# madsim-rs/madsim

Hardware: AMD Instinct MI355X
Metric: sim_seconds_per_sec (higher is better)
Workload: dtype u64

## Files before the change

madsim_amd/csrc/kernel/k_channel.h:

```cpp
#ifndef MADSIM_K_CHANNEL_H
#define MADSIM_K_CHANNEL_H

namespace madsim_k {

template <class K>
__device__ __forceinline__ int net_try_send(const Ctx& c, Lane& L, uint32_t src_node, uint32_t addr, uint32_t idx, uint64_t* latency, int* dst_sock, uint32_t* from_lb, uint32_t* dst_hdr,
                                            uint32_t known_idx = ~0u, uint32_t known_hdr = 0) {
    const KParams& P = c.P;
    int res = 0;
    uint32_t hdr = 0;
    if (K::G && PLAIN_ADDR) {
        if (idx == known_idx) {
#ifdef MADSIM_EMU
            if (known_hdr != (uint32_t)SW(c, idx, 0)) OVF_SET(L, OVF_BUG);
#endif
            hdr = known_hdr;
        } else hdr = SW(c, idx, 0);
    }
    int dn = (int)(addr & 0xff);
    if (!PLAIN_ADDR) dn = resolve_dest_node<K>(c, src_node, addr);
    if (dn >= 0) {
        const uint32_t dst_node = (uint32_t)dn;
        bool clogged = false;
        const bool mir = K::LIFE && MADSIM_CLOG_MIRROR;
        if (P.has_clog && (!mir || (L.loss_always & 0x100u))) clogged = ((CLOGW(1) >> src_node) & 1) | ((CLOGW(0) >> dst_node) & 1);
        if (P.has_clog_link && (!mir || (L.loss_always & 0x200u))) clogged |= (CLOGW(2 + src_node) >> dst_node) & 1;
        if (!clogged && !gen_bool_pint<K>(c, L, L.loss_pint, K::LIFE ? (L.loss_always & 1u) : L.loss_always)) {
            L.msg_count++;
            *latency = sample_latency<K>(c, L);
            int ds;
            if (PLAIN_ADDR) { if (!K::G) hdr = SW(c, idx, 0); ds = (hdr & 1) ? (int)idx : -1; }
            else {
                ds = find_exact<K>(c, dst_node, addr);
                if (ds < 0) ds = find_exact<K>(c, dst_node, (addr & 0xffff0000u) | (MADSIM_ADDR_UNSPECIFIED << 8));
                if (ds >= 0) hdr = SW(c, (uint32_t)ds, 0);
            }
            if (ds >= 0) {
                *from_lb = 0;
                res = 1;
                if (!PLAIN_ADDR) {
                    *from_lb = ((addr >> 8) & 0xff) == MADSIM_ADDR_LOOPBACK;
// ... 115 lines not shown
```

madsim_amd/csrc/kernel/k_lifecycle.h:

```cpp
#ifndef MADSIM_K_LIFECYCLE_H
#define MADSIM_K_LIFECYCLE_H

namespace madsim_k {

struct SpawnInit { bool parent_known; uint32_t parent_f, parent_u1y; bool move_req; uint32_t w, from, req;
                   bool words_known; uint32_t slot, w_old, w_gen, seq, w_killed; };
template <class K>
__device__ __forceinline__ uint32_t spawn_task(const Ctx& c, Lane& L, uint32_t prog, bool record, bool via_handle = false, int parent = -1,
                                               const SpawnInit init = SpawnInit{false, 0, 0, false, 0, 0, 0, false, 0, 0, 0, 0, 0}) {
    uint32_t slot = 0;
    if (K::G) {
        slot = c.P.max_tasks;
        if (init.words_known) slot = init.slot;
        else for (uint32_t wi = 0; wi < (c.P.max_tasks + 31) / 32; wi++) {
            uint32_t free_bits = ~AMASK(wi);
            if (free_bits) { slot = wi * 32 + (uint32_t)__builtin_ctz(free_bits); break; }
        }
#ifdef MADSIM_EMU
        if (init.words_known && ((AMASK(slot >> 5) >> (slot & 31)) & 1)) OVF_SET(L, OVF_BUG);
#endif
    } else {
        while (slot < c.P.max_tasks && (TWORD(c, slot, 0, 0) & TF_ALIVE)) slot++;
    }
    if (slot >= c.P.max_tasks) { OVF_SET(L, c.P.max_tasks >= MADSIM_MAX_LIVE_TASKS ? OVF_MODEL : OVF_CAP); return 0xffffffffu; }
    if (K::G) AMASK(slot >> 5) |= 1u << (slot & 31);
    uint32_t pw, node, gen, killed = 0, info_gen = 0, seq = 0;
    if constexpr (K::G) {
        pw = PROGW(c, prog);
        node = pw & 0xff;
        uint32_t w_old = init.w_old;
        uint32_t w_gen = init.w_gen, w_parent_f = init.parent_f, w_parent_y = init.parent_u1y, w_killed = init.w_killed;
        const bool in_parent = parent >= 0;
        seq = init.seq;
        if (!init.words_known) {
            w_old = TWORD(c, slot, 0, 0);
            if (K::FN) {
                w_gen = NODEW(4 + (node >> 2));
                seq = NODEW(3);
                if (!in_parent) w_killed = NODEW(via_handle ? 2u : 0u);
// ... 67 lines not shown
            uint32_t m = OMASK(wi);
            while (m) {
                uint32_t ix[4], ow[4], n = 0;
                for (uint32_t k = 0; k < 4; k++) { ix[k] = wi * 32 + (uint32_t)__builtin_ctz(m | 0x80000000u); if (m) { n++; m &= m - 1; } }
                for (uint32_t k = 0; k < 4; k++) ow[k] = SW(c, k < n ? ix[k] : ix[0], 1);
                for (uint32_t k = 0; k < 4; k++) {
                    if (k >= n || ow[k] != key) continue;
                    const uint32_t i = ix[k];
                    OMASK(i >> 5) &= ~(1u << (i & 31));
                    endpoint_drop<K>(c, L, i, (f & TF_KILLED) != 0);
                    if (SW(c, i, 1) != ~0u) SW(c, i, 1) = 0x0000ff00u;
                }
            }
        }
    } else if (f & TF_OWNER) {
        for (uint32_t i = 0; i < c.P.n_socks; i++) {
            const uint32_t hdr = SW(c, i, 0);
            if (!sock_owned_by<K>(c, i, hdr, slot, gen)) continue;
            endpoint_drop<K>(c, L, i, (f & TF_KILLED) != 0);
            if (K::LIFE && SW(c, i, 1) != ~0u) SW(c, i, 1) = 0x0000ff00u;
        }
    }
}

template <class K>
__device__ __forceinline__ void task_drop_guard(const Ctx& c, Lane& L, uint32_t slot, uint32_t prog) {
    if (K::FN && K::FA && ((PROGW(c, prog) >> 8) & MADSIM_PROG_DROP_SPAWN)) spawn_task<K>(c, L, prog + 1, false, false, (int)slot);
}

struct FinishKnown { bool have; uint32_t f, link, cx; bool have_h; uint32_t h; };
template <class K>
// ... 166 lines not shown
```

madsim_amd/csrc/kernel/k_main.h:

```cpp
#ifndef MADSIM_K_MAIN_H
#define MADSIM_K_MAIN_H

namespace madsim_k {

template <class K>
__device__ __forceinline__ void seed_init(const Ctx& c, Lane& L, uint64_t seed) {
    const KParams& P = c.P;
    if (K::G) {
        for (uint32_t w = 0; w < P.gs_plane_words; w++) gs_store32(c.gs, gs_addr_word(c, P.gs_planes + w * 4), 0);
        for (uint32_t w = 0; w < (P.max_tasks + 31) / 32; w++) AMASK(w) = 0;
        OMASK(0) = 0; OMASK(1) = 0;
        if (K::NH) for (uint32_t w = 0; w < P.pool_n / 32; w++) PMASK(w) = 0;
    }
    else for (uint32_t w = 0; w < P.lane_words; w++) RW(w) = 0;
    if (K::DEDUP) { for (uint32_t b = 0; b < P.dedup_n; b++) gs_store32(c.gs, gs_addr_uword(c, P.dedup_off + b * 16u + 12u), 0); L.hazard = 0; L.dd_occ = 0; }
    for (uint32_t t = 0; t < P.max_tasks; t++) { TWORD(c, t, 0, 0) = 0; if (!K::LIFE) TWORD(c, t, 1, 1) = 0; }
    if (K::FA && P.ipvs_dyn)
        for (uint32_t k = 0; k < P.n_services; k++) {
            const uint32_t w0 = SMEM[c.nodet0 + P.svc_off + 2 * k], w1 = SMEM[c.nodet0 + P.svc_off + 2 * k + 1];
            IPVSW(2 * k) = (w0 >> 16) | (w1 << 16);
            IPVSW(2 * k + 1) = (w1 >> 16) | (((w0 >> 8) & 7u) << 16) | ((w0 & 0x8000u) ? 0u : 1u << 24);
        }
    uint64_t x = seed, z;
#define SPLITMIX(dst) x += 0x9e3779b97f4a7c15ull; z = x; z = (z ^ (z >> 30)) * 0xbf58476d1ce4e5b9ull; z = (z ^ (z >> 27)) * 0x94d049bb133111ebull; dst = z ^ (z >> 31)
    SPLITMIX(L.s0); SPLITMIX(L.s1); SPLITMIX(L.s2); SPLITMIX(L.s3);
#undef SPLITMIX
    L.peek = rng_out(L);
    L.rng_calls = 0; L.clock = 0; L.msg_count = 0; L.steps = 0;
    L.pq_n = 0; L.ready_len = 0; L.rq = 0; L.heap_len = 0; L.top_dl = ~0ull; L.top_meta = 0; L.verdict = MADSIM_RUNNING; L.ovf = 0; L.main_done = 0;
    L.loss_pint = P.loss_pint; L.loss_always = P.loss_always;
    L.clock_fold = 0;
    { uint64_t h = L.trace_hash, n = L.log_len; uint32_t bt = gen_range_small<Variant<false, false, K::LWS, 0, K::RQ>, 31536000u>(c, L); L.trace_hash = h; L.log_len = n;
      if (K::LIFE) NODEW(4 + ((P.n_nodes + 4) >> 2)) = bt; }
    L.trace_hash = FNV_OFFSET; L.obs_hash = FNV_OFFSET; L.log_len = 0;
    if (K::TRACE) L.obs_len = 0;
    for (uint32_t p = 1; p < P.n_progs; p++) {
        uint32_t fl = (PROGW(c, p) >> 8) & 0xff;
        if (fl & MADSIM_PROG_PRE) spawn_task<K>(c, L, p, !(fl & MADSIM_PROG_INIT));
    }
    spawn_task<K>(c, L, 0, true);
}

#ifndef MADSIM_G_WAVES_PER_EU
#define MADSIM_G_WAVES_PER_EU 3
#endif
#ifndef MADSIM_ALLG_WAVES_PER_EU
#define MADSIM_ALLG_WAVES_PER_EU 2
#endif
constexpr uint32_t MADSIM_PRIO_EVERY_MASK = 15u;
__device__ __forceinline__ uint32_t progress_priority(uint32_t pass, uint32_t est) {
    const uint32_t q = (pass < (1u << 30) ? pass : (1u << 30) - 1u) * 4u / est;
    return q >= 3 ? 0u : 3u - q;
}

template <class K> struct PopOne { static constexpr bool ON = MADSIM_POP_ONE && K::RQ; };

template <class K>
__global__ __launch_bounds__(256, K::CMP ? 4 : !K::G ? 1 : (K::FEAT & (MADSIM_FEAT_ALL & ~MADSIM_FEAT_ADDR)) == (MADSIM_FEAT_ALL & ~MADSIM_FEAT_ADDR) ? MADSIM_ALLG_WAVES_PER_EU : MADSIM_G_WAVES_PER_EU) void sim_kernel(const KParams P) {
    const uint32_t lane = threadIdx.x & 63, wv = threadIdx.x >> 6;
    uint32_t* sh = SMEM;
    const uint32_t cp0 = table_copy_first(), cps = table_copy_stride(P.waves_per_block);
    for (uint32_t i = cp0; i < P.n_insns * 4; i += cps) sh[P.sh_insns + i] = ((const uint32_t*)P.insns)[i];
    for (uint32_t i = cp0; i < P.n_progs; i += cps) sh[P.sh_progs + i] = P.progs[i];
    for (uint32_t i = cp0; i < P.n_socks; i += cps) sh[P.sh_socks + i] = P.socks[i];
    for (uint32_t i = cp0; i < P.n_nodetab; i += cps) sh[P.sh_nodes + i] = P.nodes[i];
    __syncthreads();

    Ctx c(P);
    c.insn0 = P.sh_insns / 4;
    c.prog0 = P.sh_progs;
    c.sockt0 = P.sh_socks;
    c.nodet0 = P.sh_nodes;
    const uint32_t wbase = wv * P.wave_words;
    if (K::NH) c.heap0 = (P.sh_heap + wbase) / 2 + lane;
    else if (K::LIFE) c.heap0 = (P.sh_heap + wbase) / 4 + lane;
    else if (K::CMP) { c.heap0 = (P.sh_heap + wbase) / 2 + lane; c.heapm0 = 0; }
    else { c.heap0 = (P.sh_heap + wbase) / 2 + lane; c.heapm0 = P.sh_heap + wbase + ((P.heap_lds * 2) << P.lw_shift) + lane; }
    c.lws = P.lw_shift;
    const uint32_t pl = P.sh_planes + wbase + lane;
    c.ready0 = pl + (P.off_ready << P.lw_shift);
    c.amask0 = pl + (P.off_amask << P.lw_shift);
    c.omask0 = pl + (P.off_omask << P.lw_shift);
    c.pmask0 = pl + (P.off_pmask << P.lw_shift);
    if (K::G) {
        c.task0 = 0;
        c.sock0 = P.gs_planes + P.off_socks * 4; c.hand0 = P.gs_planes + P.off_handles * 4; c.node0 = P.gs_planes + P.off_nodes * 4;
        c.clog0 = P.gs_planes + P.off_clog * 4; c.pause0 = P.gs_planes + P.off_pause * 4; c.greg0 = P.gs_planes + P.off_greg * 4;
        c.conn0 = P.gs_planes + P.off_conn * 4; c.hook0 = P.gs_planes + P.off_hooks * 4; c.ipvs0 = P.gs_planes + P.off_ipvs * 4;
    } else {
        c.task0 = (P.sh_tasks + wbase) / 4 + lane;
        c.task1 = (P.sh_tasks + wbase + ((P.max_tasks * 4) << P.lw_shift)) / 2 + lane;
        if (K::CMP) {
            c.task1 = (P.sh_tasks + wbase + (((P.max_tasks - 1) * 4) << P.lw_shift)) / 2 + lane - (1u << P.lw_shift);
// ... 17 lines not shown
    c.gs_lane = glane;
    c.gs = buf_make(P.gstate, (uint64_t)P.gs_stride * P.total_lanes);
    c.tlog = P.trace_log;

    Lane L;
#ifdef MADSIM_K_PROF
    for (int i = 0; i < 12; i++) L.prof_acc[i] = 0;
    L.prof_t = __builtin_readcyclecounter(); uint64_t prof_iters = 0;
#endif
    L.exact = 0; L.hazard = 0;
    uint64_t next = glane;
    bool have = false;
    uint32_t pass_est = (K::TRACE || !P.iter_est) ? 0u : wave_uniform(*P.iter_est);
    uint32_t pass = 0;
    for (;;) {
        if (!K::TRACE && P.iter_est) {
            const uint32_t pu = wave_uniform(pass);
            if ((pu & MADSIM_PRIO_EVERY_MASK) == 0) {
                if (!pass_est && (pu & 63u) == 0) pass_est = wave_uniform(__atomic_load_n(P.iter_est, __ATOMIC_RELAXED));
                if (pass_est) wave_set_priority(progress_priority(pu, pass_est));
            }
        }
        pass++;
        if (!have) {
            if (next >= P.count) break;
            if (K::TRACE) {
                c.tlog = P.trace_log + next * P.trace_cap;
                c.olog = (P.obs_log && P.obs_cap) ? P.obs_log + next * P.obs_cap : nullptr;
            }
            seed_init<K>(c, L, P.seed_list ? P.seed_list[next] : P.seed0 + next);
            have = true;
        }
#ifdef MADSIM_K_PROF
        prof_iters++;
#endif
        uint64_t now = L.clock;
        PROBE(0);
        REG(0);
        if (L.ready_len > 0) {
            const uint32_t slot0 = K::RQ ? (uint32_t)(L.rq & 0xff) : rq_get<K>(c, 0);
            const uint4 pu0 = TU(c, slot0, 0), pu1 = load_u1<K>(c, slot0);
            PollPrefetch pp = poll_prefetch<K>(c, slot0);
            if (ClockFold<K>::ON) L.clock_fold = clock_fold_byte(L.clock);
            const bool all_one = wave_all(L.ready_len == 1);
            uint32_t idx = gen_index<K>(c, L, L.ready_len, all_one);
// ... 84 lines not shown
            }
            L.verdict = v;
            if (v != MADSIM_RUNNING || more) break;
            now = L.top_dl + 50;
            idle_jump = true;
        }
        PROBE(4);
        if (K::DEDUP && L.hazard) { L.exact = 1; have = false; continue; }
        if (L.ovf) L.verdict = (L.ovf & OVF_CAP) ? MADSIM_OVERFLOW : (L.ovf & OVF_BUG) ? MADSIM_INTERNAL : MADSIM_UNSUPPORTED;
        if (L.verdict != MADSIM_RUNNING) {
            REG(25);
            madsim_result_t r;
            r.verdict = L.verdict; r.steps = L.steps; r.clock_ns = L.clock; r.msg_count = L.msg_count;
            r.rng_calls = L.rng_calls; r.trace_hash = (K::NOLOG || (K::LOGSW && P.no_log)) ? 0 : L.trace_hash; r.obs_hash = L.obs_hash;
            if (r.verdict >= MADSIM_UNSUPPORTED) { r.steps = 0; r.clock_ns = 0; r.msg_count = 0; r.rng_calls = 0; r.trace_hash = 0; r.obs_hash = 0; }
            P.out[next] = r;
            if (K::TRACE) { P.trace_len[next] = L.log_len; if (P.obs_len) P.obs_len[next] = L.obs_len; }
            have = false;
            if (K::DEDUP) L.exact = 0;
            if (P.work_ctr) next = P.total_lanes + atomicAdd(P.work_ctr, 1ull);
            else next += P.total_lanes / EXP_LANE_DIV;
        }
    }
    if (!K::TRACE && P.iter_est) {
        if (K::LIFE) {
            const uint32_t wmax = wave_max_u32(pass);
            if (wave_first_lane() && wmax > 16) atomic_max_u32(P.iter_est, wmax);
        } else if (lane == 0 && pass > 16) *P.iter_est = pass;
    }
#ifdef MADSIM_K_PROF
    PROBE2(0);
    if (lane == 0 && P.prof) { for (int i = 0; i < 12; i++) atomicAdd((unsigned long long*)&P.prof[i], (unsigned long long)L.prof_acc[i]); atomicAdd((unsigned long long*)&P.prof[12], (unsigned long long)prof_iters); atomicAdd((unsigned long long*)&P.prof[13], 1ull); }
#endif
}

}

#endif
```

madsim_amd/csrc/kernel/k_poll.h:

```cpp
#ifndef MADSIM_K_POLL_H
#define MADSIM_K_POLL_H

namespace madsim_k {

__device__ __forceinline__ uint64_t sleep_deadline(const Lane& L, uint64_t deadline) {
    uint64_t m = L.clock + NS_PER_MS;
    return deadline > m ? deadline : m;
}

template <class K>
__device__ __forceinline__ uint64_t rand_delay_deadline(const Ctx& c, Lane& L) {
    uint64_t delay = (uint64_t)gen_range_small<K, 5>(c, L) * 1000ull;
    if (c.P.buggify) {
        if (gen_bool_pint<K>(c, L, c.P.bug_pint, 0)) delay = (uint64_t)(1 + gen_range_small<K, 4>(c, L)) * NS_PER_S;
    }
    return sleep_deadline(L, L.clock + delay);
}

__device__ __forceinline__ uint64_t loss_pint_at(const KParams& P, uint32_t i) {
    i &= 3;
    return i == 0 ? P.loss_table_pint[0] : i == 1 ? P.loss_table_pint[1] : i == 2 ? P.loss_table_pint[2] : P.loss_table_pint[3];
}
__device__ __forceinline__ uint32_t loss_always_at(const KParams& P, uint32_t i) {
    i &= 3;
    return i == 0 ? P.loss_table_always[0] : i == 1 ? P.loss_table_always[1] : i == 2 ? P.loss_table_always[2] : P.loss_table_always[3];
}

__device__ __forceinline__ bool may_have_twin(uint32_t flags, uint32_t gen) { return (flags & TF_RXWRAP) || gen > 0xff; }
// ... 46 lines not shown
        u0.w = MADSIM_VAL_TIMEOUT;
        return true;
    }
    timer_schedule<K>(c, L, dl, (EV_WAKE << EV_SHIFT) | (gen << 8) | slot, 0, true, again);
    return false;
}

__device__ __forceinline__ bool is_light(uint32_t op) {
    return op == MS_OP_ASSERT_VAL || op == MS_OP_DJNZ || op == MS_OP_SET || op == MS_OP_JMP || op == MS_OP_TRACE || op == MS_OP_JEQ;
}

template <class K>
__device__ __forceinline__ bool poll_task(const Ctx& c, Lane& L, const uint32_t slot, uint4& u0, uint4 u1, PollPrefetch pp) {
    enum : uint32_t { ST_RUN = 0, ST_PENDING = 1, ST_FINISHED = 2, ST_PANIC = 3 };
    const KParams& P = c.P;
    const uint32_t REGS_FULL = P.mbox_regs >= MADSIM_MAX_MBOX_REGS ? (uint32_t)OVF_MODEL : (uint32_t)OVF_CAP;
    bool u1_dirty = false;
    uint32_t pc = u0.y & 0xffff, sub = (u0.y >> 16) & 0xff, from = u0.y >> 24;
    const uint32_t gen = (u0.x >> 8) & 0xffff;
    const uint32_t node = PROGW(c, u0.x >> 24) & 0xff;
    uint32_t st = ST_RUN;
    bool sig = false;
    if constexpr (K::FSIG) { sig = (sub & SUB_SIGNALLED) != 0; sub &= ~SUB_SIGNALLED; }

    bool first_poll = false;
    constexpr bool CU_FULL = Hoist<K>::CHAN;
    auto cu_get = [&]() -> uint4 { if (CU_FULL) return pp.cu; return (uint4)TU(c, slot, c.P.chan_unit); };
    auto cu0_get = [&]() -> uint32_t { if (K::G) return pp.cu.x; return (uint32_t)TWORD(c, slot, c.P.chan_unit, 0); };
    auto cu0_set = [&](uint32_t v) { if (K::G) pp.cu.x = v; TWORD(c, slot, c.P.chan_unit, 0) = v; };
    auto cu_set = [&](const uint4& v) { if (CU_FULL) pp.cu = v; else if (K::G) pp.cu.x = v.x; TU(c, slot, c.P.chan_unit) = v; };
#ifdef MADSIM_EMU
// ... 627 lines not shown
                    if (K::FR && P.uses_rpc && (b & MADSIM_SPAWN_MOVE_REQUEST) && child != 0xffffffffu) {
                        TWORD(c, child, 0, 3) = u0.w;
                        TWORD(c, child, 0, 1) = (TWORD(c, child, 0, 1) & 0x00ffffffu) | (from << 24);
                        TWORD(c, child, P.rpc_unit, 0) = TWORD(c, slot, P.rpc_unit, 0);
                    }
                }
                if (K::FC && P.uses_chan && (b & 2) && child != 0xffffffffu) {
                    uint32_t cx = cu0_get();
                    TWORD(c, child, c.P.chan_unit, 0) = cx & 0x1ff;
                    cu0_set(cx | 0xff);
                }
            }
                pc++;
                break;
            case MS_OP_BUILD:
                for (uint32_t p = 1; p < P.n_progs; p++) {
                    uint32_t pw = PROGW(c, p);
                    if ((pw & 0xff) == a && ((pw >> 8) & MADSIM_PROG_INIT) && !((pw >> 8) & MADSIM_PROG_PRE)) spawn_task<K>(c, L, p, false);
                }
                pc++;
                break;
            case MS_OP_JOIN: {
                uint32_t hs;
                if (sub == SUB_JOIN_WAIT) { st = ST_PENDING; break; }
                if (sub != 0) { hs = sub == SUB_JOIN_CANCELLED ? H_CANCELLED : H_COMPLETED; sub = 0; }
                else {
                    const uint32_t h = HW(a);
                    hs = h & 3;
                    if (hs == H_RUNNING) {
                        const uint32_t cs = (h >> 8) & 0xff;
                        const uint32_t link = TWORD(c, cs, 1, 0);
// ... 294 lines not shown
            REG(17);
            u1.z = (uint32_t)deadline; u1.w = (uint32_t)(deadline >> 32); u1_dirty = true;
            sub = (op == MS_OP_RECV) ? 3 : 1;
            timer_schedule<K>(c, L, deadline, (EV_WAKE << EV_SHIFT) | (gen << 8) | slot, 0, true);
            st = ST_PENDING;
        }
    }
    PROBE(9);
    if (st != ST_FINISHED) {
        u0.y = pc | (sub << 16) | (from << 24);
        if (u1_dirty) tu1_store<K>(c, slot, u1);
    }
    return st == ST_PANIC;
}
#undef RX_DROP
#undef SCOPE_DROP_CONN

}

#endif
```

madsim_amd/csrc/kernel/k_state.h:

```cpp
#ifndef MADSIM_K_STATE_H
#define MADSIM_K_STATE_H

namespace madsim_k {

#ifdef MADSIM_EXPERIMENT_BUILD
#include <type_traits>
#include "../../../tools/experiment/k_experiment.h"
#else
#if defined(EXP_NOLOG) || defined(EXP_ALWAYS_ACCEPT) || defined(EXP_PROF) || defined(EXP_PROF2) || defined(EXP_NO_LWS_VARIANTS) || defined(EXP_HALF_LANES)
#error "EXP_* switches make a non-bit-exact kernel: build experiment variants with tools/build_variant.sh, never the product Makefile"
#endif
#define EXP_ACCEPT(x) (x)
#define EXP_LANE_DIV 1u
#define MADSIM_K_LOG_ENABLED 1
#define PROBE(i) do { } while (0)
#define PROBE2(i) do { } while (0)
#define PROBE_FLUSH() do { } while (0)
#endif
#define FNV_OFFSET 14695981039346656037ull
#define FNV_PRIME 1099511628211ull
#define NS_PER_S 1000000000ull
#define NS_PER_MS 1000000ull

enum : uint32_t { TF_ALIVE = 1, TF_SCHED = 2, TF_RUN = 4, TF_KILLED = 8, TF_CANCEL = 16, TF_INBOX = 32,
// ... 14 lines not shown
    static constexpr int LWS = LWS_, FEAT = FEAT_ & MADSIM_FEAT_ALL;
    static constexpr bool LIFE = FEAT != 0;
    static constexpr bool CMP = (FEAT_ & MADSIM_FEAT_COMPACT) != 0;
    static constexpr bool NOLOG = (FEAT_ & MADSIM_FEAT_NOLOG) != 0;
    static constexpr bool NH = (FEAT_ & MADSIM_FEAT_NARROW) != 0;
    static constexpr bool LOGSW = !NOLOG && !TRACE_ && (LIFE || SPILL_ || LWS_ != 6);
    static constexpr bool DEDUP = G_ && !TRACE_ && (FEAT_ & MADSIM_FEAT_ALL) == MADSIM_FEAT_TIME;
    static constexpr bool FT = (FEAT_ & MADSIM_FEAT_TIME) != 0, FC = (FEAT_ & MADSIM_FEAT_CHAN) != 0,
                          FR = (FEAT_ & MADSIM_FEAT_RPC) != 0, FN = (FEAT_ & MADSIM_FEAT_NODE) != 0,
                          FA = (FEAT_ & MADSIM_FEAT_ADDR) != 0;
    static constexpr bool FS = (FEAT_ & MADSIM_FEAT_SCOPE) != 0;
    static constexpr bool FK = (FEAT_ & MADSIM_FEAT_TICK) != 0;
    static constexpr bool FSEL = (FEAT_ & MADSIM_FEAT_SELECT) != 0;
    static constexpr bool FSIG = (FEAT_ & MADSIM_FEAT_SIGNAL) != 0;
};

#ifndef REG
#define REG(id) do { } while (0)
#endif

enum : uint32_t { OVF_CAP = 1, OVF_MODEL = 2, OVF_BUG = 4 };
#ifdef MADSIM_EMU
void madsim_emu_ovf_note(const char* file, int line, uint32_t bits);
#define OVF_SET(L, bits) ((L).ovf = (L).ovf ? (L).ovf : (bits), madsim_emu_ovf_note(__FILE__, __LINE__, (bits)))
#else
#define OVF_SET(L, bits) ((L).ovf = (L).ovf ? (L).ovf : (bits))
#endif
struct Lane {
    uint64_t s0, s1, s2, s3;
    uint64_t peek;
// ... 37 lines not shown
    uint32_t sock0;
    uint32_t heap0;
    uint32_t heapm0;
    uint32_t task0;
    uint32_t task1;
    uint32_t insn0;
    uint32_t prog0, sockt0, nodet0;
    BufRef spill;
    uint32_t spill_off;
    BufRef gs;
    uint32_t gs_lane;
    uint32_t amask0, omask0;
    uint32_t pmask0;
    uint8_t* tlog;
    uint64_t* olog;
    __device__ Ctx(const KParams& p) : P(p) {}
};

template <class K> __device__ __forceinline__ uint32_t LWSH(const Ctx& c) { return K::LWS >= 0 ? (uint32_t)K::LWS : c.lws; }
#define RW(i) SMEM[c.ready0 + ((i) << LWSH<K>(c))]
template <class K> __device__ __forceinline__ uint32_t rq_get(const Ctx& c, uint32_t i) {
    if (!K::G) return RW(i);
    return (RW(i >> 2) >> ((i & 3u) * 8u)) & 0xffu;
}
template <class K> __device__ __forceinline__ void rq_set(const Ctx& c, uint32_t i, uint32_t slot) {
    if (!K::G) { RW(i) = slot; return; }
    const uint32_t sh = (i & 3u) * 8u, w = RW(i >> 2);
    RW(i >> 2) = (w & ~(0xffu << sh)) | (slot << sh);
}
#define AMASK(i) SMEM[c.amask0 + ((i) << LWSH<K>(c))]
#define OMASK(i) SMEM[c.omask0 + ((i) << LWSH<K>(c))]
#define PMASK(i) SMEM[c.pmask0 + ((i) << LWSH<K>(c))]

// ... 25 lines not shown
    __device__ __forceinline__ uint32_t operator+=(uint32_t v) const { return *this = (uint32_t)*this + v; }
};
template <bool G> struct URef;
template <> struct URef<false> {
    uint32_t at;
    __device__ __forceinline__ operator uint4() const { return LDS128(at); }
    __device__ __forceinline__ void operator=(const uint4& v) const { LDS128(at) = v; }
    __device__ __forceinline__ void operator=(const URef& o) const { *this = (uint4)o; }
};
template <> struct URef<true> {
    BufRef gs; uint32_t at;
    __device__ __forceinline__ operator uint4() const { return gs_load128(gs, at); }
    __device__ __forceinline__ void operator=(const uint4& v) const { gs_store128(gs, at, v); }
    __device__ __forceinline__ void operator=(const URef& o) const { *this = (uint4)o; }
};
struct HWRef {
    BufRef gs; uint32_t at; bool glob;
    __device__ __forceinline__ operator uint32_t() const { uint32_t v; if (glob) v = gs_load32(gs, at); else v = SMEM[at]; return v; }
    __device__ __forceinline__ uint32_t operator=(uint32_t v) const { if (glob) gs_store32(gs, at, v); else SMEM[at] = v; return v; }
    __device__ __forceinline__ uint32_t operator=(const HWRef& o) const { return *this = (uint32_t)o; }
    __device__ __forceinline__ uint32_t operator|=(uint32_t v) const { return *this = (uint32_t)*this | v; }
    __device__ __forceinline__ uint32_t operator&=(uint32_t v) const { return *this = (uint32_t)*this & v; }
    __device__ __forceinline__ uint32_t operator+=(uint32_t v) const { return *this = (uint32_t)*this + v; }
};
struct HURef {
    BufRef gs; uint32_t at; bool glob;
    __device__ __forceinline__ operator uint4() const { uint4 v; if (glob) v = gs_load128(gs, at); else v = LDS128(at); return v; }
    __device__ __forceinline__ void operator=(const uint4& v) const { if (glob) gs_store128(gs, at, v); else LDS128(at) = v; }
    __device__ __forceinline__ void operator=(const HURef& o) const { *this = (uint4)o; }
};
template <class K> struct TaskRef {
    typedef typename std::conditional<K::CMP, HURef, URef<K::G>>::type U;
    typedef typename std::conditional<K::CMP, HWRef, WRef<K::G>>::type W;
};
template <bool G> __device__ __forceinline__ WRef<G> make_wref(const Ctx& c, uint32_t lds_at, uint32_t gs_at);
template <> __device__ __forceinline__ WRef<false> make_wref<false>(const Ctx&, uint32_t lds_at, uint32_t) { return WRef<false>{lds_at}; }
__device__ __forceinline__ uint32_t gs_addr_unit(const Ctx& c, uint32_t at) { return __umul24(at, c.P.total_lanes) + c.gs_lane * 16u; }
__device__ __forceinline__ uint32_t gs_addr_uword(const Ctx& c, uint32_t at) { return __umul24(at & ~15u, c.P.total_lanes) + c.gs_lane * 16u + (at & 15u); }
__device__ __forceinline__ uint32_t gs_addr_word(const Ctx& c, uint32_t at) { return __umul24(at, c.P.total_lanes) + c.gs_lane * 4u; }
template <> __device__ __forceinline__ WRef<true> make_wref<true>(const Ctx& c, uint32_t, uint32_t gs_at) { return WRef<true>{c.gs, gs_addr_word(c, gs_at)}; }
__device__ __forceinline__ WRef<true> make_uword_ref(const Ctx& c, uint32_t gs_at) { return WRef<true>{c.gs, gs_addr_uword(c, gs_at)}; }
template <bool G> __device__ __forceinline__ URef<G> make_uref(const Ctx& c, uint32_t lds_at, uint32_t gs_at);
template <> __device__ __forceinline__ URef<false> make_uref<false>(const Ctx&, uint32_t lds_at, uint32_t) { return URef<false>{lds_at}; }
template <> __device__ __forceinline__ URef<true> make_uref<true>(const Ctx& c, uint32_t, uint32_t gs_at) { return URef<true>{c.gs, gs_addr_unit(c, gs_at)}; }
template <class K> __device__ __forceinline__ WRef<K::G> plane_ref(const Ctx& c, uint32_t base, uint32_t i) {
    return make_wref<K::G>(c, base + (i << LWSH<K>(c)), base + i * 4u);
}
#define NODEW(i) plane_ref<K>(c, c.node0, (i))
// ... 27 lines not shown
template <> __device__ __forceinline__ URef<false> tu_gs<false>(const Ctx&, uint32_t, uint32_t) { return URef<false>{0}; }
template <> __device__ __forceinline__ URef<true> tu_gs<true>(const Ctx& c, uint32_t slot, uint32_t u) { return URef<true>{c.gs, gs_addr_task(c, slot, u * 16u)}; }
template <bool G> __device__ __forceinline__ WRef<G> tword_gs2(const Ctx& c, uint32_t slot, uint32_t u, uint32_t k);
template <> __device__ __forceinline__ WRef<false> tword_gs2<false>(const Ctx&, uint32_t, uint32_t, uint32_t) { return WRef<false>{0}; }
template <> __device__ __forceinline__ WRef<true> tword_gs2<true>(const Ctx& c, uint32_t slot, uint32_t u, uint32_t k) { return WRef<true>{c.gs, gs_addr_task(c, slot, u * 16u + k * 4u)}; }
template <class K> __device__ __forceinline__ URef<K::G> tu_ref_plain(const Ctx& c, uint32_t slot, uint32_t u) {
    if (!K::LIFE) return make_uref<K::G>(c, c.task0 + (slot << LWSH<K>(c)), 0);
    if (K::G) return tu_gs<K::G>(c, slot, u);
    return make_uref<K::G>(c, c.task0 + ((slot * c.P.task_units + u) << LWSH<K>(c)), 0);
}
template <class K> __device__ __forceinline__ WRef<K::G> tword_ref_plain(const Ctx& c, uint32_t slot, uint32_t u, uint32_t k) {
    if (!K::LIFE) return make_wref<K::G>(c, u == 0 ? (c.task0 + (slot << LWSH<K>(c))) * 4u + k : (c.task1 + (slot << LWSH<K>(c))) * 2u + k, 0);
    if (K::G) return tword_gs2<K::G>(c, slot, u, k);
    return make_wref<K::G>(c, (c.task0 + ((slot * c.P.task_units + u) << LWSH<K>(c))) * 4u + k, 0);
}
template <class K> __device__ __forceinline__ typename TaskRef<K>::U tu_ref(const Ctx& c, uint32_t slot, uint32_t u) {
    if constexpr (K::CMP) return HURef{c.gs, slot == 0 ? c.gs_lane * 16u : c.task0 + (slot << LWSH<K>(c)), slot == 0};
    else return tu_ref_plain<K>(c, slot, u);
}
template <class K> __device__ __forceinline__ typename TaskRef<K>::W tword_ref(const Ctx& c, uint32_t slot, uint32_t u, uint32_t k) {
    if constexpr (K::CMP) {
        const uint32_t lds = u == 0 ? (c.task0 + (slot << LWSH<K>(c))) * 4u + k : (c.task1 + (slot << LWSH<K>(c))) * 2u + k;
        const uint32_t glb = u == 0 ? c.gs_lane * 16u + k * 4u : c.P.total_lanes * 16u + c.gs_lane * 8u + k * 4u;
        return HWRef{c.gs, slot == 0 ? glb : lds, slot == 0};
    } else return tword_ref_plain<K>(c, slot, u, k);
}
template <class K> __device__ __forceinline__ uint4 load_u1(const Ctx& c, uint32_t slot) {
    if (K::LIFE) return tu_ref<K>(c, slot, 1);
    uint2 t;
    if (K::CMP && slot == 0) t = buf_load64(c.gs, c.P.total_lanes * 16u + c.gs_lane * 8u);
    else t = LDS64(c.task1 + (slot << LWSH<K>(c)));
    return make_uint4(t.x, t.y, 0, 0);
}
template <class K> struct Hoist {
    static constexpr bool ALLG = K::G && (K::FEAT & (MADSIM_FEAT_ALL & ~MADSIM_FEAT_ADDR)) == (MADSIM_FEAT_ALL & ~MADSIM_FEAT_ADDR);
    static constexpr bool CHAN = (K::G && K::FEAT == MADSIM_FEAT_CHAN) || ALLG;
};
struct PollPrefetch { uint32_t d2lo, d2hi; uint4 cu; uint32_t rq0, rq1; };
template <class K> struct HoistRpc { static constexpr bool ON = K::G && K::FR; };
template <class K> struct HdrPrefetch { static constexpr bool ON = Hoist<K>::ALLG && !K::FA; };
#ifndef MADSIM_RECV_PREFETCH_TIME
#define MADSIM_RECV_PREFETCH_TIME 0
#endif
template <class K> struct RecvPrefetch { static constexpr bool ON = Hoist<K>::ALLG || (MADSIM_RECV_PREFETCH_TIME && K::G && (K::FEAT & MADSIM_FEAT_ALL) == MADSIM_FEAT_TIME); };
#ifndef MADSIM_SWITCH_PREFETCH_CHAN
// ... 49 lines not shown
```

madsim_amd/csrc/sim_kernel.h:

```cpp
#ifndef MADSIM_SIM_KERNEL_H
#define MADSIM_SIM_KERNEL_H

#include <stdint.h>

#include "../../include/madsim_hip.h"

#define MADSIM_RUNNING 0xffu

#define MADSIM_FEAT_TIME 1
#define MADSIM_FEAT_CHAN 2
#define MADSIM_FEAT_RPC  4
#define MADSIM_FEAT_NODE 8
#define MADSIM_FEAT_ADDR 16
#define MADSIM_FEAT_ALL  31
#define MADSIM_FEAT_NOLOG 32
#define MADSIM_FEAT_COMPACT 64
#define MADSIM_FEAT_NARROW 128
#define MADSIM_FEAT_SCOPE 256
#define MADSIM_FEAT_TICK 512
#define MADSIM_FEAT_SELECT 1024
#define MADSIM_FEAT_TIERS (MADSIM_FEAT_SCOPE | MADSIM_FEAT_TICK | MADSIM_FEAT_SELECT)
#define MADSIM_FEAT_SIGNAL 2048
#ifndef MADSIM_FIRE_COPIES
#define MADSIM_FIRE_COPIES 2
#endif
#ifndef MADSIM_RNG_PEEK
#define MADSIM_RNG_PEEK 2
#endif
#ifndef MADSIM_RNG_PEEK_LIFE
#define MADSIM_RNG_PEEK_LIFE 0
#endif
#ifndef MADSIM_CLOCK_FOLD
#define MADSIM_CLOCK_FOLD 1
#endif
#ifndef MADSIM_POP_ONE
#define MADSIM_POP_ONE 1
#endif
#ifndef MADSIM_DEDUP_OCC
#define MADSIM_DEDUP_OCC 1
#endif
#ifndef MADSIM_CLOG_MIRROR
#define MADSIM_CLOG_MIRROR 1
#endif
#ifndef MADSIM_POP_TOPDOWN
#define MADSIM_POP_TOPDOWN 1
#endif
#ifndef MADSIM_PUSH_PREFETCH
#define MADSIM_PUSH_PREFETCH 0
#endif
#ifndef MADSIM_POP_LDS_FIRST
#define MADSIM_POP_LDS_FIRST 1
// ... 295 lines not shown
```

Before: 117.9 million.

## Re-read cold kernel parameters from kernarg segment to cut scalar register pressure

Adds a MADSIM_COLD_PARAMS mode, on by default for non-LIFE variants. Rarely used KParams fields (loop bounds, seed list, output pointers, iter_est, and the main task buffer descriptor in compact mode) are re-loaded from the kernarg segment pointer at each use instead of staying live in SGPRs. Three boolean flags (clog, clog_link, buggify) are packed into one uniform uflags word held in Ctx. The goal is lower scalar register pressure and less spilling in the large kernel, at the cost of extra scalar loads on cold paths and reliance on the kernarg layout matching offsetof(KParams).

```diff
diff --git a/madsim_amd/csrc/kernel/k_channel.h b/madsim_amd/csrc/kernel/k_channel.h
--- a/madsim_amd/csrc/kernel/k_channel.h
+++ b/madsim_amd/csrc/kernel/k_channel.h
@@ -23,8 +23,8 @@
         const uint32_t dst_node = (uint32_t)dn;
         bool clogged = false;
         const bool mir = K::LIFE && MADSIM_CLOG_MIRROR;
-        if (P.has_clog && (!mir || (L.loss_always & 0x100u))) clogged = ((CLOGW(1) >> src_node) & 1) | ((CLOGW(0) >> dst_node) & 1);
-        if (P.has_clog_link && (!mir || (L.loss_always & 0x200u))) clogged |= (CLOGW(2 + src_node) >> dst_node) & 1;
+        if (uflag<K>(c, P.has_clog, UF_CLOG) && (!mir || (L.loss_always & 0x100u))) clogged = ((CLOGW(1) >> src_node) & 1) | ((CLOGW(0) >> dst_node) & 1);
+        if (uflag<K>(c, P.has_clog_link, UF_CLOG_LINK) && (!mir || (L.loss_always & 0x200u))) clogged |= (CLOGW(2 + src_node) >> dst_node) & 1;
         if (!clogged && !gen_bool_pint<K>(c, L, L.loss_pint, K::LIFE ? (L.loss_always & 1u) : L.loss_always)) {
             L.msg_count++;
             *latency = sample_latency<K>(c, L);
diff --git a/madsim_amd/csrc/kernel/k_lifecycle.h b/madsim_amd/csrc/kernel/k_lifecycle.h
--- a/madsim_amd/csrc/kernel/k_lifecycle.h
+++ b/madsim_amd/csrc/kernel/k_lifecycle.h
@@ -9,6 +9,7 @@
 __device__ __forceinline__ uint32_t spawn_task(const Ctx& c, Lane& L, uint32_t prog, bool record, bool via_handle = false, int parent = -1,
                                                const SpawnInit init = SpawnInit{false, 0, 0, false, 0, 0, 0, false, 0, 0, 0, 0, 0}) {
     uint32_t slot = 0;
+    const KParams& P = c.P;
     if (K::G) {
         slot = c.P.max_tasks;
         if (init.words_known) slot = init.slot;
@@ -20,9 +21,10 @@
         if (init.words_known && ((AMASK(slot >> 5) >> (slot & 31)) & 1)) OVF_SET(L, OVF_BUG);
 #endif
     } else {
-        while (slot < c.P.max_tasks && (TWORD(c, slot, 0, 0) & TF_ALIVE)) slot++;
-    }
-    if (slot >= c.P.max_tasks) { OVF_SET(L, c.P.max_tasks >= MADSIM_MAX_LIVE_TASKS ? OVF_MODEL : OVF_CAP); return 0xffffffffu; }
+        const uint32_t n = ColdParams<K>::ON ? PCOLD(max_tasks) : 0u;
+        while (slot < (ColdParams<K>::ON ? n : c.P.max_tasks) && (TWORD(c, slot, 0, 0) & TF_ALIVE)) slot++;
+    }
+    if (slot >= PCOLD(max_tasks)) { OVF_SET(L, PCOLD(max_tasks) >= MADSIM_MAX_LIVE_TASKS ? OVF_MODEL : OVF_CAP); return 0xffffffffu; }
     if (K::G) AMASK(slot >> 5) |= 1u << (slot & 31);
     uint32_t pw, node, gen, killed = 0, info_gen = 0, seq = 0;
     if constexpr (K::G) {
@@ -120,7 +122,8 @@
             }
         }
     } else if (f & TF_OWNER) {
-        for (uint32_t i = 0; i < c.P.n_socks; i++) {
+        const KParams& P = c.P;
+        PCOLD_FOR(i, 0, n_socks) {
             const uint32_t hdr = SW(c, i, 0);
             if (!sock_owned_by<K>(c, i, hdr, slot, gen)) continue;
             endpoint_drop<K>(c, L, i, (f & TF_KILLED) != 0);
diff --git a/madsim_amd/csrc/kernel/k_main.h b/madsim_amd/csrc/kernel/k_main.h
--- a/madsim_amd/csrc/kernel/k_main.h
+++ b/madsim_amd/csrc/kernel/k_main.h
@@ -12,9 +12,9 @@
         OMASK(0) = 0; OMASK(1) = 0;
         if (K::NH) for (uint32_t w = 0; w < P.pool_n / 32; w++) PMASK(w) = 0;
     }
-    else for (uint32_t w = 0; w < P.lane_words; w++) RW(w) = 0;
+    else PCOLD_FOR(w, 0, lane_words) RW(w) = 0;
     if (K::DEDUP) { for (uint32_t b = 0; b < P.dedup_n; b++) gs_store32(c.gs, gs_addr_uword(c, P.dedup_off + b * 16u + 12u), 0); L.hazard = 0; L.dd_occ = 0; }
-    for (uint32_t t = 0; t < P.max_tasks; t++) { TWORD(c, t, 0, 0) = 0; if (!K::LIFE) TWORD(c, t, 1, 1) = 0; }
+    PCOLD_FOR(t, 0, max_tasks) { TWORD(c, t, 0, 0) = 0; if (!K::LIFE) TWORD(c, t, 1, 1) = 0; }
     if (K::FA && P.ipvs_dyn)
         for (uint32_t k = 0; k < P.n_services; k++) {
             const uint32_t w0 = SMEM[c.nodet0 + P.svc_off + 2 * k], w1 = SMEM[c.nodet0 + P.svc_off + 2 * k + 1];
@@ -28,13 +28,13 @@
     L.peek = rng_out(L);
     L.rng_calls = 0; L.clock = 0; L.msg_count = 0; L.steps = 0;
     L.pq_n = 0; L.ready_len = 0; L.rq = 0; L.heap_len = 0; L.top_dl = ~0ull; L.top_meta = 0; L.verdict = MADSIM_RUNNING; L.ovf = 0; L.main_done = 0;
-    L.loss_pint = P.loss_pint; L.loss_always = P.loss_always;
+    L.loss_pint = PCOLD(loss_pint); L.loss_always = PCOLD(loss_always);
     L.clock_fold = 0;
     { uint64_t h = L.trace_hash, n = L.log_len; uint32_t bt = gen_range_small<Variant<false, false, K::LWS, 0, K::RQ>, 31536000u>(c, L); L.trace_hash = h; L.log_len = n;
       if (K::LIFE) NODEW(4 + ((P.n_nodes + 4) >> 2)) = bt; }
     L.trace_hash = FNV_OFFSET; L.obs_hash = FNV_OFFSET; L.log_len = 0;
     if (K::TRACE) L.obs_len = 0;
-    for (uint32_t p = 1; p < P.n_progs; p++) {
+    PCOLD_FOR(p, 1, n_progs) {
         uint32_t fl = (PROGW(c, p) >> 8) & 0xff;
         if (fl & MADSIM_PROG_PRE) spawn_task<K>(c, L, p, !(fl & MADSIM_PROG_INIT));
     }
@@ -57,6 +57,7 @@
 
 template <class K>
 __global__ __launch_bounds__(256, K::CMP ? 4 : !K::G ? 1 : (K::FEAT & (MADSIM_FEAT_ALL & ~MADSIM_FEAT_ADDR)) == (MADSIM_FEAT_ALL & ~MADSIM_FEAT_ADDR) ? MADSIM_ALLG_WAVES_PER_EU : MADSIM_G_WAVES_PER_EU) void sim_kernel(const KParams P) {
+    static_assert(std::is_same<decltype(&sim_kernel<K>), void (*)(KParams)>::value && std::is_trivially_copyable<KParams>::value, "PCOLD: KParams by value, alone");
     const uint32_t lane = threadIdx.x & 63, wv = threadIdx.x >> 6;
     uint32_t* sh = SMEM;
     const uint32_t cp0 = table_copy_first(), cps = table_copy_stride(P.waves_per_block);
@@ -77,6 +78,7 @@
     else if (K::CMP) { c.heap0 = (P.sh_heap + wbase) / 2 + lane; c.heapm0 = 0; }
     else { c.heap0 = (P.sh_heap + wbase) / 2 + lane; c.heapm0 = P.sh_heap + wbase + ((P.heap_lds * 2) << P.lw_shift) + lane; }
     c.lws = P.lw_shift;
+    c.uflags = ColdParams<K>::ON ? uflags_word(P) : 0u;
     const uint32_t pl = P.sh_planes + wbase + lane;
     c.ready0 = pl + (P.off_ready << P.lw_shift);
     c.amask0 = pl + (P.off_amask << P.lw_shift);
@@ -124,21 +126,21 @@
     uint32_t pass_est = (K::TRACE || !P.iter_est) ? 0u : wave_uniform(*P.iter_est);
     uint32_t pass = 0;
     for (;;) {
-        if (!K::TRACE && P.iter_est) {
+        if (!K::TRACE && (ColdParams<K>::ON || P.iter_est)) {
             const uint32_t pu = wave_uniform(pass);
-            if ((pu & MADSIM_PRIO_EVERY_MASK) == 0) {
-                if (!pass_est && (pu & 63u) == 0) pass_est = wave_uniform(__atomic_load_n(P.iter_est, __ATOMIC_RELAXED));
+            if ((pu & MADSIM_PRIO_EVERY_MASK) == 0 && (!ColdParams<K>::ON || PCOLD(iter_est))) {
+                if (!pass_est && (pu & 63u) == 0) pass_est = wave_uniform(__atomic_load_n(PCOLD(iter_est), __ATOMIC_RELAXED));
                 if (pass_est) wave_set_priority(progress_priority(pu, pass_est));
             }
         }
         pass++;
         if (!have) {
-            if (next >= P.count) break;
+            if (next >= PCOLD(count)) break;
             if (K::TRACE) {
                 c.tlog = P.trace_log + next * P.trace_cap;
                 c.olog = (P.obs_log && P.obs_cap) ? P.obs_log + next * P.obs_cap : nullptr;
             }
-            seed_init<K>(c, L, P.seed_list ? P.seed_list[next] : P.seed0 + next);
+            { const uint64_t* const sl = PCOLD(seed_list); seed_init<K>(c, L, sl ? sl[next] : PCOLD(seed0) + next); }
             have = true;
         }
 #ifdef MADSIM_K_PROF
@@ -253,19 +255,19 @@
             r.verdict = L.verdict; r.steps = L.steps; r.clock_ns = L.clock; r.msg_count = L.msg_count;
             r.rng_calls = L.rng_calls; r.trace_hash = (K::NOLOG || (K::LOGSW && P.no_log)) ? 0 : L.trace_hash; r.obs_hash = L.obs_hash;
             if (r.verdict >= MADSIM_UNSUPPORTED) { r.steps = 0; r.clock_ns = 0; r.msg_count = 0; r.rng_calls = 0; r.trace_hash = 0; r.obs_hash = 0; }
-            P.out[next] = r;
+            PCOLD(out)[next] = r;
             if (K::TRACE) { P.trace_len[next] = L.log_len; if (P.obs_len) P.obs_len[next] = L.obs_len; }
             have = false;
             if (K::DEDUP) L.exact = 0;
-            if (P.work_ctr) next = P.total_lanes + atomicAdd(P.work_ctr, 1ull);
-            else next += P.total_lanes / EXP_LANE_DIV;
-        }
-    }
-    if (!K::TRACE && P.iter_est) {
+            if (unsigned long long* const wc = PCOLD(work_ctr)) next = PCOLD(total_lanes) + atomicAdd(wc, 1ull);
+            else next += PCOLD(total_lanes) / EXP_LANE_DIV;
+        }
+    }
+    if (!K::TRACE && PCOLD(iter_est)) {
         if (K::LIFE) {
             const uint32_t wmax = wave_max_u32(pass);
             if (wave_first_lane() && wmax > 16) atomic_max_u32(P.iter_est, wmax);
-        } else if (lane == 0 && pass > 16) *P.iter_est = pass;
+        } else if (lane == 0 && pass > 16) *PCOLD(iter_est) = pass;
     }
 #ifdef MADSIM_K_PROF
     PROBE2(0);
diff --git a/madsim_amd/csrc/kernel/k_poll.h b/madsim_amd/csrc/kernel/k_poll.h
--- a/madsim_amd/csrc/kernel/k_poll.h
+++ b/madsim_amd/csrc/kernel/k_poll.h
@@ -11,7 +11,7 @@
 template <class K>
 __device__ __forceinline__ uint64_t rand_delay_deadline(const Ctx& c, Lane& L) {
     uint64_t delay = (uint64_t)gen_range_small<K, 5>(c, L) * 1000ull;
-    if (c.P.buggify) {
+    if (uflag<K>(c, c.P.buggify, UF_BUGGIFY)) {
         if (gen_bool_pint<K>(c, L, c.P.bug_pint, 0)) delay = (uint64_t)(1 + gen_range_small<K, 4>(c, L)) * NS_PER_S;
     }
     return sleep_deadline(L, L.clock + delay);
@@ -88,7 +88,8 @@
 __device__ __forceinline__ bool poll_task(const Ctx& c, Lane& L, const uint32_t slot, uint4& u0, uint4 u1, PollPrefetch pp) {
     enum : uint32_t { ST_RUN = 0, ST_PENDING = 1, ST_FINISHED = 2, ST_PANIC = 3 };
     const KParams& P = c.P;
-    const uint32_t REGS_FULL = P.mbox_regs >= MADSIM_MAX_MBOX_REGS ? (uint32_t)OVF_MODEL : (uint32_t)OVF_CAP;
+    const uint32_t regs_full_hot = P.mbox_regs >= MADSIM_MAX_MBOX_REGS ? (uint32_t)OVF_MODEL : (uint32_t)OVF_CAP;
+#define REGS_FULL (ColdParams<K>::ON ? (PCOLD(mbox_regs) >= MADSIM_MAX_MBOX_REGS ? (uint32_t)OVF_MODEL : (uint32_t)OVF_CAP) : regs_full_hot)
     bool u1_dirty = false;
     uint32_t pc = u0.y & 0xffff, sub = (u0.y >> 16) & 0xff, from = u0.y >> 24;
     const uint32_t gen = (u0.x >> 8) & 0xffff;
@@ -746,7 +747,7 @@
                 pc++;
                 break;
             case MS_OP_BUILD:
-                for (uint32_t p = 1; p < P.n_progs; p++) {
+                PCOLD_FOR(p, 1, n_progs) {
                     uint32_t pw = PROGW(c, p);
                     if ((pw & 0xff) == a && ((pw >> 8) & MADSIM_PROG_INIT) && !((pw >> 8) & MADSIM_PROG_PRE)) spawn_task<K>(c, L, p, false);
                 }
@@ -1071,6 +1072,7 @@
     return st == ST_PANIC;
 }
 #undef RX_DROP
+#undef REGS_FULL
 #undef SCOPE_DROP_CONN
 
 }
diff --git a/madsim_amd/csrc/kernel/k_state.h b/madsim_amd/csrc/kernel/k_state.h
--- a/madsim_amd/csrc/kernel/k_state.h
+++ b/madsim_amd/csrc/kernel/k_state.h
@@ -52,6 +52,32 @@
     static constexpr bool FSEL = (FEAT_ & MADSIM_FEAT_SELECT) != 0;
     static constexpr bool FSIG = (FEAT_ & MADSIM_FEAT_SIGNAL) != 0;
 };
+
+#ifdef MADSIM_EMU
+template <class K> struct ColdParams { static constexpr bool ON = false; };
+#define PCOLD(f) (P.f)
+#else
+template <class K> struct ColdParams { static constexpr bool ON = MADSIM_COLD_PARAMS && !K::LIFE; };
+template <bool ON, class T> __device__ __forceinline__ T cold_read(const T& hot, uint32_t off) {
+    if constexpr (ON) {
+        typedef const char __attribute__((address_space(4)))* seg_t;
+        seg_t p = (seg_t)__builtin_amdgcn_kernarg_segment_ptr();
+        asm volatile("" : "+s"(p));
+        return *(const T __attribute__((address_space(4)))*)(p + off);
+    } else return hot;
+}
+#define PCOLD(f) cold_read<ColdParams<K>::ON>(P.f, (uint32_t)offsetof(KParams, f))
+#endif
+#define PCOLD_FOR(i_, start_, f_) for (uint32_t i_ = (start_), i_##_n = ColdParams<K>::ON ? PCOLD(f_) : 0u; i_ < (ColdParams<K>::ON ? i_##_n : P.f_); i_++)
+enum : uint32_t { UF_CLOG = 1, UF_CLOG_LINK = 2, UF_BUGGIFY = 4 };
+__device__ __forceinline__ uint32_t uflags_word(const KParams& P) {
+    uint32_t f = (P.has_clog ? (uint32_t)UF_CLOG : 0u) | (P.has_clog_link ? (uint32_t)UF_CLOG_LINK : 0u) | (P.buggify ? (uint32_t)UF_BUGGIFY : 0u);
+#ifndef MADSIM_EMU
+    f = wave_uniform(f);
+    asm volatile("" : "+s"(f));
+#endif
+    return f;
+}
 
 #ifndef REG
 #define REG(id) do { } while (0)
@@ -119,9 +145,20 @@
     uint32_t pmask0;
     uint8_t* tlog;
     uint64_t* olog;
+    uint32_t uflags;
     __device__ Ctx(const KParams& p) : P(p) {}
 };
 
+template <class K> __device__ __forceinline__ bool uflag(const Ctx& c, uint32_t hot, uint32_t bit) {
+#ifndef MADSIM_EMU
+    if constexpr (ColdParams<K>::ON) {
+        uint32_t f = c.uflags;
+        asm volatile("" : "+s"(f));
+        return (f & bit) != 0;
+    } else
+#endif
+    return hot != 0;
+}
 template <class K> __device__ __forceinline__ uint32_t LWSH(const Ctx& c) { return K::LWS >= 0 ? (uint32_t)K::LWS : c.lws; }
 #define RW(i) SMEM[c.ready0 + ((i) << LWSH<K>(c))]
 template <class K> __device__ __forceinline__ uint32_t rq_get(const Ctx& c, uint32_t i) {
@@ -177,24 +214,33 @@
     __device__ __forceinline__ void operator=(const uint4& v) const { gs_store128(gs, at, v); }
     __device__ __forceinline__ void operator=(const URef& o) const { *this = (uint4)o; }
 };
-struct HWRef {
-    BufRef gs; uint32_t at; bool glob;
-    __device__ __forceinline__ operator uint32_t() const { uint32_t v; if (glob) v = gs_load32(gs, at); else v = SMEM[at]; return v; }
-    __device__ __forceinline__ uint32_t operator=(uint32_t v) const { if (glob) gs_store32(gs, at, v); else SMEM[at] = v; return v; }
+struct NoBuf { };
+template <bool COLD> struct MainBuf { typedef BufRef T; static __device__ __forceinline__ const BufRef& get(const BufRef& b) { return b; } };
+#ifndef MADSIM_EMU
+__device__ __forceinline__ BufRef main_task_buf() {
+    return buf_make(cold_read<true, uint8_t*>(nullptr, (uint32_t)offsetof(KParams, gstate)),
+                    (uint64_t)cold_read<true, uint32_t>(0u, (uint32_t)offsetof(KParams, gs_stride)) * cold_read<true, uint32_t>(0u, (uint32_t)offsetof(KParams, total_lanes)));
+}
+template <> struct MainBuf<true> { typedef NoBuf T; static __device__ __forceinline__ BufRef get(const NoBuf&) { return main_task_buf(); } };
+#endif
+template <bool COLD> struct HWRef {
+    typename MainBuf<COLD>::T gs; uint32_t at; bool glob;
+    __device__ __forceinline__ operator uint32_t() const { uint32_t v; if (glob) v = gs_load32(MainBuf<COLD>::get(gs), at); else v = SMEM[at]; return v; }
+    __device__ __forceinline__ uint32_t operator=(uint32_t v) const { if (glob) gs_store32(MainBuf<COLD>::get(gs), at, v); else SMEM[at] = v; return v; }
     __device__ __forceinline__ uint32_t operator=(const HWRef& o) const { return *this = (uint32_t)o; }
     __device__ __forceinline__ uint32_t operator|=(uint32_t v) const { return *this = (uint32_t)*this | v; }
     __device__ __forceinline__ uint32_t operator&=(uint32_t v) const { return *this = (uint32_t)*this & v; }
     __device__ __forceinline__ uint32_t operator+=(uint32_t v) const { return *this = (uint32_t)*this + v; }
 };
-struct HURef {
-    BufRef gs; uint32_t at; bool glob;
-    __device__ __forceinline__ operator uint4() const { uint4 v; if (glob) v = gs_load128(gs, at); else v = LDS128(at); return v; }
-    __device__ __forceinline__ void operator=(const uint4& v) const { if (glob) gs_store128(gs, at, v); else LDS128(at) = v; }
+template <bool COLD> struct HURef {
+    typename MainBuf<COLD>::T gs; uint32_t at; bool glob;
+    __device__ __forceinline__ operator uint4() const { uint4 v; if (glob) v = gs_load128(MainBuf<COLD>::get(gs), at); else v = LDS128(at); return v; }
+    __device__ __forceinline__ void operator=(const uint4& v) const { if (glob) gs_store128(MainBuf<COLD>::get(gs), at, v); else LDS128(at) = v; }
     __device__ __forceinline__ void operator=(const HURef& o) const { *this = (uint4)o; }
 };
 template <class K> struct TaskRef {
-    typedef typename std::conditional<K::CMP, HURef, URef<K::G>>::type U;
-    typedef typename std::conditional<K::CMP, HWRef, WRef<K::G>>::type W;
+    typedef typename std::conditional<K::CMP, HURef<ColdParams<K>::ON>, URef<K::G>>::type U;
+    typedef typename std::conditional<K::CMP, HWRef<ColdParams<K>::ON>, WRef<K::G>>::type W;
 };
 template <bool G> __device__ __forceinline__ WRef<G> make_wref(const Ctx& c, uint32_t lds_at, uint32_t gs_at);
 template <> __device__ __forceinline__ WRef<false> make_wref<false>(const Ctx&, uint32_t lds_at, uint32_t) { return WRef<false>{lds_at}; }
@@ -252,21 +298,24 @@
     if (K::G) return tword_gs2<K::G>(c, slot, u, k);
     return make_wref<K::G>(c, (c.task0 + ((slot * c.P.task_units + u) << LWSH<K>(c))) * 4u + k, 0);
 }
+template <class K> __device__ __forceinline__ typename MainBuf<ColdParams<K>::ON>::T main_buf_of(const Ctx& c) {
+    if constexpr (ColdParams<K>::ON) return NoBuf{}; else return c.gs;
+}
 template <class K> __device__ __forceinline__ typename TaskRef<K>::U tu_ref(const Ctx& c, uint32_t slot, uint32_t u) {
-    if constexpr (K::CMP) return HURef{c.gs, slot == 0 ? c.gs_lane * 16u : c.task0 + (slot << LWSH<K>(c)), slot == 0};
+    if constexpr (K::CMP) return HURef<ColdParams<K>::ON>{main_buf_of<K>(c), slot == 0 ? c.gs_lane * 16u : c.task0 + (slot << LWSH<K>(c)), slot == 0};
     else return tu_ref_plain<K>(c, slot, u);
 }
 template <class K> __device__ __forceinline__ typename TaskRef<K>::W tword_ref(const Ctx& c, uint32_t slot, uint32_t u, uint32_t k) {
     if constexpr (K::CMP) {
         const uint32_t lds = u == 0 ? (c.task0 + (slot << LWSH<K>(c))) * 4u + k : (c.task1 + (slot << LWSH<K>(c))) * 2u + k;
         const uint32_t glb = u == 0 ? c.gs_lane * 16u + k * 4u : c.P.total_lanes * 16u + c.gs_lane * 8u + k * 4u;
-        return HWRef{c.gs, slot == 0 ? glb : lds, slot == 0};
+        return HWRef<ColdParams<K>::ON>{main_buf_of<K>(c), slot == 0 ? glb : lds, slot == 0};
     } else return tword_ref_plain<K>(c, slot, u, k);
 }
 template <class K> __device__ __forceinline__ uint4 load_u1(const Ctx& c, uint32_t slot) {
     if (K::LIFE) return tu_ref<K>(c, slot, 1);
     uint2 t;
-    if (K::CMP && slot == 0) t = buf_load64(c.gs, c.P.total_lanes * 16u + c.gs_lane * 8u);
+    if (K::CMP && slot == 0) { const KParams& P = c.P; t = buf_load64(MainBuf<ColdParams<K>::ON>::get(main_buf_of<K>(c)), PCOLD(total_lanes) * 16u + c.gs_lane * 8u); }
     else t = LDS64(c.task1 + (slot << LWSH<K>(c)));
     return make_uint4(t.x, t.y, 0, 0);
 }
diff --git a/madsim_amd/csrc/sim_kernel.h b/madsim_amd/csrc/sim_kernel.h
--- a/madsim_amd/csrc/sim_kernel.h
+++ b/madsim_amd/csrc/sim_kernel.h
@@ -35,6 +35,9 @@
 #endif
 #ifndef MADSIM_POP_ONE
 #define MADSIM_POP_ONE 1
+#endif
+#ifndef MADSIM_COLD_PARAMS
+#define MADSIM_COLD_PARAMS 1
 #endif
 #ifndef MADSIM_DEDUP_OCC
 #define MADSIM_DEDUP_OCC 1
```

New measurement: 119.9 million, median of 6. 1.7% higher.
